# spcl/EBCC

Measured on AMD Instinct MI355X. Metric: fp32 GB/s encode+decode, 721x1440 ERA5 frames MAX_ERROR=0.5, higher is better.
Workload: dtype f32; 1 GPU; 256-frame batch 721x1440 fp32 per GPU, base_cr=30 MAX_ERROR=0.5 (BASELINE configs[1]); frames_per_gpu=256, parallelism=frames sharded over 1 GPU(s), no collective, hw_queues=4, encode_slices=3

## Files before the change

### ebcc_amd/csrc/j2k.hip

```cpp
#include <algorithm>
#include <cstring>
#include <vector>

#include "../../include/ebcc_hip.h"
#include "engine.hpp"
#include "j2k.hpp"

namespace ebcc {

bool j2k_create(ebcc_hip_ctx *ctx)
{
    J2kBuffers *jb = new J2kBuffers();
    ctx->j2k = jb;
    const int period = ctx->tile_period;
    std::vector<std::vector<J2kBlock>> tile_blocks((size_t) period);
    int stride = 0;
    for (int k = 0; k < period; k++) {
        jb->geoms.push_back(make_j2k_geom(ctx->height, ctx->width, tile_blocks[(size_t) k], k * ctx->height));
        stride = std::max(stride, jb->geoms.back().nblocks);
    }
    for (J2kGeom &t : jb->geoms) { t.period = period; t.stride = stride; }
    jb->geom = jb->geoms[0];
    const J2kGeom &g = jb->geom;
    const size_t n_pix = ctx->n_pix, F = ctx->max_frames;
    const size_t total = F * (size_t) stride, groups = (total + 63) / 64;
    jb->max_frames = (int) F;
    jb->fs = ctx->rb.fs;
    jb->stream_cap = ((n_pix * 3 + 4096 + 63) / 64) * 64;
    bool ok = true;
    ok &= (jb->d_geom = (J2kGeom *) ctx_alloc<uint8_t>(ctx, sizeof(J2kGeom) * (size_t) period)) != nullptr;
    ok &= (jb->d_blocks = (J2kBlock *) ctx_alloc<uint8_t>(ctx, sizeof(J2kBlock) * (size_t) period * (size_t) stride)) != nullptr;
    ok &= (jb->d_blkmap = ctx_alloc<uint16_t>(ctx, (size_t) period * n_pix)) != nullptr;
    ok &= (jb->B = ctx_alloc<float>(ctx, F * n_pix)) != nullptr;
    ok &= (jb->B2 = ctx_alloc<float>(ctx, F * n_pix)) != nullptr;
    ok &= (jb->Q6 = ctx_alloc<int32_t>(ctx, F * n_pix)) != nullptr;
    ok &= (jb->DEC = ctx_alloc<float>(ctx, F * n_pix)) != nullptr;
    ok &= (jb->V = ctx_alloc<int32_t>(ctx, F * n_pix)) != nullptr;
    ok &= (jb->BP = ctx_alloc<unsigned long long>(ctx, groups * kJ2kMaxPlanes * 64 * 64)) != nullptr;
    ok &= (jb->SGN = ctx_alloc<unsigned long long>(ctx, groups * 64 * 64)) != nullptr;
    ok &= (jb->SUF = ctx_alloc<unsigned long long>(ctx, groups * (kJ2kMaxPlanes + 2) * 64 * 64)) != nullptr;
    ok &= (jb->SPS = ctx_alloc<unsigned long long>(ctx, groups * 64 * 64)) != nullptr;
    ok &= (jb->VISP = ctx_alloc<unsigned long long>(ctx, groups * kJ2kMaxPlanes * 64 * 64)) != nullptr;
    ok &= (jb->ckpt = ctx_alloc<uint8_t>(ctx, groups * 64 * j2k_ckpt_block_bytes())) != nullptr;
    jb->SYM = nullptr;
    {
        const char *e = getenv("EBCC_T1_TWO_PHASE");
        jb->sym_rows = kJ2kSymRows;
        if (const char *r = getenv("EBCC_HIP_SYM_ROWS")) jb->sym_rows = std::max(1, std::min(kJ2kSymRows, atoi(r)));
        if (!e || atoi(e)) ok &= (jb->SYM = ctx_alloc<uint8_t>(ctx, groups * (size_t) ((jb->sym_rows + 1) & ~1) * 1024 + 256)) != nullptr;
    }
    ok &= (jb->seglen = ctx_alloc<uint16_t>(ctx, groups * (size_t) kJ2kSegCount * 64)) != nullptr;
    ok &= (jb->lanerows = ctx_alloc<uint32_t>(ctx, groups * 64)) != nullptr;
    ok &= (jb->qplane = (int *) ctx_alloc<int32_t>(ctx, groups * 64)) != nullptr;
    ok &= (jb->lastnp = (int *) ctx_alloc<int32_t>(ctx, groups * 64)) != nullptr;
    ok &= (jb->T1S = ctx_alloc<unsigned long long>(ctx, groups * kT1StateWords * 64)) != nullptr;
    ok &= (jb->blkmax = (int *) ctx_alloc<int32_t>(ctx, groups * 64)) != nullptr;
    ok &= (jb->numbps = (int *) ctx_alloc<int32_t>(ctx, groups * 64)) != nullptr;
    ok &= (jb->totalpasses = (int *) ctx_alloc<int32_t>(ctx, groups * 64)) != nullptr;
    ok &= (jb->cblk_len = (int *) ctx_alloc<int32_t>(ctx, groups * 64)) != nullptr;
    ok &= (jb->npass = (int *) ctx_alloc<int32_t>(ctx, groups * 64)) != nullptr;
    ok &= (jb->cand_cr = ctx_alloc<float>(ctx, F * 2)) != nullptr;
    ok &= (jb->cand_out = (int *) ctx_alloc<int32_t>(ctx, F * 6)) != nullptr;
    ok &= (jb->cand_npass = (int *) ctx_alloc<int32_t>(ctx, 2 * F * (size_t) stride)) != nullptr;
    ok &= (jb->cand_sel = (int *) ctx_alloc<int32_t>(ctx, F)) != nullptr;
    ok &= (jb->have_rate = (int *) ctx_alloc<int32_t>(ctx, F)) != nullptr;
    ok &= (jb->rate_path = (int *) ctx_alloc<int32_t>(ctx, F * 1536 * 3)) != nullptr;
    ok &= (jb->rate_path_n = (int *) ctx_alloc<int32_t>(ctx, 2 * F)) != nullptr;
    {
        int nodes = 0;
        for (const J2kGeom &t : jb->geoms) nodes = std::max(nodes, t.tree_nodes);
        J2kBuffers::RateCache &rc = jb->rate_cache;
        rc.nodes_cap = (nodes + 3) & ~3;
        rc.cap = stride * kJ2kMaxPasses;
        rc.ok = jb->rate_path_n ? jb->rate_path_n + F : nullptr;
        ok &= (rc.mnmx = ctx_alloc<double>(ctx, F * 2)) != nullptr;
        ok &= (rc.mval = (short *) ctx_alloc<uint16_t>(ctx, F * (size_t) rc.nodes_cap)) != nullptr;
        ok &= (rc.off = (int *) ctx_alloc<int32_t>(ctx, F * (size_t) (stride + 1))) != nullptr;
        ok &= (rc.crate = ctx_alloc<uint16_t>(ctx, F * (size_t) rc.cap)) != nullptr;
        ok &= (rc.cdisto = ctx_alloc<double>(ctx, F * (size_t) rc.cap)) != nullptr;
    }
    ok &= (jb->rates = (int *) ctx_alloc<int32_t>(ctx, groups * 64 * kJ2kMaxPasses)) != nullptr;
    ok &= (jb->disto = ctx_alloc<double>(ctx, groups * 64 * kJ2kMaxPasses)) != nullptr;
    ok &= (jb->cblk_bytes = ctx_alloc<uint8_t>(ctx, groups * 64 * kJ2kCblkBytes)) != nullptr;
    ok &= (jb->stream = ctx_alloc<uint8_t>(ctx, F * jb->stream_cap)) != nullptr;
    ok &= (jb->dec_table = (int *) ctx_alloc<int32_t>(ctx, groups * 64 * 4)) != nullptr;
    ok &= (jb->dec_order = (int *) ctx_alloc<int32_t>(ctx, groups * 64 + 128)) != nullptr;
    ok &= (jb->mq_order = (int *) ctx_alloc<int32_t>(ctx, groups * 64 + 256)) != nullptr;
    ok &= (jb->jf = (J2kFrame *) ctx_alloc<uint8_t>(ctx, sizeof(J2kFrame) * F)) != nullptr;
    ok &= (jb->partial = ctx_alloc<double>(ctx, F * kPartials)) != nullptr;
    ok &= (jb->partial_u = ctx_alloc<unsigned long long>(ctx, F * kPartials)) != nullptr;
    if (!ok) return false;
    poison_alloc(jb->cblk_bytes, groups * 64 * kJ2kCblkBytes);
    poison_alloc(jb->stream, F * jb->stream_cap);
    if (stride >= 65535) { set_error("too many code-blocks"); return false; }
    std::vector<uint16_t> map((size_t) period * n_pix, 0);
    std::vector<J2kBlock> blocks((size_t) period * (size_t) stride, J2kBlock{});
    for (int k = 0; k < period; k++) {
        const std::vector<J2kBlock> &tb = tile_blocks[(size_t) k];
        std::copy(tb.begin(), tb.end(), blocks.begin() + (size_t) k * (size_t) stride);
        for (size_t b = 0; b < tb.size(); b++)
            for (int y = 0; y < tb[b].h; y++)
                for (int x = 0; x < tb[b].w; x++) map[(size_t) k * n_pix + (size_t) (tb[b].y + y) * g.W + tb[b].x + x] = (uint16_t) b;
    }
    hipStream_t s = ctx->stream;
    EBCC_HIP_CHECK(hipMemcpyAsync(jb->d_geom, jb->geoms.data(), sizeof(J2kGeom) * (size_t) period, hipMemcpyHostToDevice, s));
    EBCC_HIP_CHECK(hipMemcpyAsync(jb->d_blocks, blocks.data(), sizeof(J2kBlock) * blocks.size(), hipMemcpyHostToDevice, s));
    EBCC_HIP_CHECK(hipMemcpyAsync(jb->d_blkmap, map.data(), map.size() * sizeof(uint16_t), hipMemcpyHostToDevice, s));
    EBCC_HIP_CHECK(hipHostMalloc(&ctx->h_jf, sizeof(J2kFrame) * F));
    EBCC_HIP_CHECK(hipHostMalloc((void **) &ctx->h_table, sizeof(int) * 4 * total));
    EBCC_HIP_CHECK(hipMemsetAsync(jb->jf, 0, sizeof(J2kFrame) * F, s));
    EBCC_HIP_CHECK(hipMemsetAsync(jb->rate_path_n, 0, sizeof(int) * 2 * F, s));
    wait_stream(s);
    return true;
}

void j2k_destroy(ebcc_hip_ctx *ctx)
{
    delete static_cast<J2kBuffers *>(ctx->j2k);
    ctx->j2k = nullptr;
    if (ctx->stream2) { hipStreamSynchronize(ctx->stream2); hipStreamDestroy(ctx->stream2); ctx->stream2 = nullptr; }
}

namespace {

struct BitReader {
    const uint8_t *p, *end;
// ... 478 lines not shown
```

### ebcc_amd/csrc/j2k.hpp

```cpp
#pragma once

#include <vector>

#include "../../include/ebcc_hip.h"
#include "common.hpp"
#include "residual.hpp"

namespace ebcc {

constexpr int kJ2kRes = 6;
constexpr int kJ2kBands = 3 * kJ2kRes - 2;
constexpr int kJ2kMaxPlanes = 26;
constexpr int kJ2kMaxPasses = 3 * kJ2kMaxPlanes;
constexpr int kJ2kCblkBytes = 16 * 1024;
constexpr int kT1StateWords = 66 + 4 * 64;

struct J2kBand {
    int res, orient, level;
    int x0, y0, x1, y1;
    int offx, offy;
    int ncw, nch;
    int first_block;
    int expn, mant, numbps;
    float step_enc, step_dec;
// ... 52 lines not shown
    float target;
    int maxlen;
    int body_bytes;
    int stream_bytes;
    unsigned long long nbad;
    double err_sum;
    int overflow;
    int keep;
    float hdr_share;
    unsigned int bad_limit;
    unsigned int bad_seen;
};

struct J2kBuffers {
    J2kGeom geom;
    std::vector<J2kGeom> geoms;
    J2kGeom *d_geom;
    J2kBlock *d_blocks;
    std::uint16_t *d_blkmap;
    int max_frames;
    float *B;
    float *B2;
    int32_t *Q6;
    float *DEC;
    unsigned long long *BP;
    unsigned long long *SGN;
    unsigned long long *SUF;
    unsigned long long *SPS;
    unsigned long long *VISP;
    void *ckpt;
    uint8_t *SYM;
    int sym_rows;
    std::uint16_t *seglen;
    std::uint32_t *lanerows;
    int *qplane;
    int *lastnp;
    unsigned long long *T1S;
    int *blkmax;
    int *numbps;
    int *totalpasses;
    int *cblk_len;
    int *rates;
    double *disto;
    int *npass;
    float *cand_cr;
    int *cand_out;
    int *cand_npass;
    int *cand_sel;
    int *have_rate;
    int *rate_path;
    int *rate_path_n;
    struct RateCache {
        int *ok;
        double *mnmx;
        short *mval;
        int *off;
        unsigned short *crate;
        double *cdisto;
        int nodes_cap, cap;
    } rate_cache;
    uint8_t *cblk_bytes;
    uint8_t *stream;
    size_t stream_cap;
    int32_t *V;
    int *dec_table;
    int *dec_order;
// ... 74 lines not shown
```

### ebcc_amd/csrc/j2k_analysis.hip

```cpp
#include <array>
#include <mutex>
#include <cmath>
#include <cstdlib>
#include <vector>

#include "j2k.hpp"
#include "t1_core.hpp"
#include "t1_device.hpp"

namespace ebcc {

static int ceildivpow2(int a, int b) { return (int) (((long long) a + (1ll << b) - 1) >> b); }
static int floorlog2i(int a) { int l = 0; while (a > 1) { a >>= 1; l++; } return l; }

static const double kNormsReal[4][10] = {
    {1.000, 1.965, 4.177, 8.403, 16.90, 33.84, 67.69, 135.3, 270.6, 540.9},
    {2.022, 3.989, 8.355, 17.04, 34.27, 68.63, 137.3, 274.6, 549.0},
    {2.022, 3.989, 8.355, 17.04, 34.27, 68.63, 137.3, 274.6, 549.0},
    {2.080, 3.865, 8.307, 17.18, 34.71, 69.59, 139.3, 278.6, 557.2}};

int t1_lanes_per_wave(int kernel, int total_blocks)
{
    int t[4] = {64, 64, 4, 2};
    if (const char *e = getenv("EBCC_T1_LPW")) {
// ... 1087 lines not shown

struct DevMasks {
    const unsigned char *bp, *suf, *sg;
    unsigned char *visp;
    uint32_t lane8;
    __device__ unsigned long long ld(const unsigned char *b, int row) const { return *(const unsigned long long *) (b + ((uint32_t) row * 512u + lane8)); }
    __device__ unsigned long long BP(int p, int y) const { return ld(bp, p * 64 + y); }
    __device__ unsigned long long SUF(int p, int y) const { return ld(suf, p * 64 + y); }
    __device__ unsigned long long SGN(int y) const { return ld(sg, y); }
    __device__ unsigned long long VISP(int p, int y) const { return ld(visp, p * 64 + y); }
};
struct Tier1Lane {
    int gid, frame, P, w, h, orient;
    bool live;
};
__device__ inline Tier1Lane tier1_lane(int gid, int total, const int *blkmax, const J2kGeom *geom, const J2kBlock *blocks, const FrameState *fs)
{
    Tier1Lane l{gid, 0, 0, 0, 0, 0, false};
    if (gid >= total) return l;
    const int nb = geom->stride;
    l.frame = gid / nb;
    if (fs[l.frame].const_field) return l;
    const J2kBlock blk = j2k_frame_blocks(geom, blocks, l.frame)[gid - l.frame * nb];
    const int m = blkmax[gid];
    l.P = m ? (31 - __clz(m)) + 1 - 6 : 0;
    l.w = blk.w; l.h = blk.h;
    l.orient = j2k_frame_geom(geom, l.frame).bands[blk.band].orient;
    l.live = l.P > 0;
    return l;
}

struct ScanOutDev {
    unsigned char *vp, *sp;
    std::uint16_t *lens;
    uint32_t lane8;
    __device__ void visp_row(unsigned char *b, int row, unsigned long long v) const { *(unsigned long long *) (b + ((uint32_t) row * 512u + lane8)) = v; }
    __device__ void visp(int p, int y, unsigned long long m) const { visp_row(vp, p * 64 + y, m); }
    __device__ void sps_or(int y, unsigned long long n) const { *(unsigned long long *) (sp + ((uint32_t) y * 512u + lane8)) |= n; }
    __device__ void len(int seg, uint32_t n) const { lens[(uint32_t) seg * 64u] = (std::uint16_t) n; }
};
__global__ __launch_bounds__(64) void k_t1_scan(const unsigned long long *BP, const unsigned long long *SUF, const unsigned long long *SGN,
                                                 unsigned long long *SPS, unsigned long long *VISP, const int *blkmax, int *numbps,
                                                 int *totalpasses, int *cblk_len, std::uint16_t *seglen, const J2kGeom *geom,
                                                 const J2kBlock *blocks, const FrameState *fs, int total)
{
    const size_t grp = blockIdx.x;
    const int gid = (int) (grp * 64) + (int) threadIdx.x;
    const Tier1Lane l = tier1_lane(gid, total, blkmax, geom, blocks, fs);
    if (gid < total) { numbps[gid] = l.P; totalpasses[gid] = l.live ? 3 * l.P - 2 : 0; cblk_len[gid] = 0; }
    if (!l.live) return;
    const uint32_t lane8 = threadIdx.x * 8u;
    DevMasks M{(const unsigned char *) (BP + grp * kJ2kMaxPlanes * 64 * 64), (const unsigned char *) (SUF + grp * (kJ2kMaxPlanes + 2) * 64 * 64),
               (const unsigned char *) (SGN + grp * 64 * 64), (unsigned char *) (VISP + grp * kJ2kMaxPlanes * 64 * 64), lane8};
    ScanOutDev out{M.visp, (unsigned char *) (SPS + grp * 64 * 64), seglen + grp * kJ2kSegCount * 64 + threadIdx.x, lane8};
    t1::scan_block(M, out, l.P, l.w, l.h, l.orient);
}

__global__ __launch_bounds__(64) void k_t1_rowoffs(std::uint16_t *seglen, uint32_t *lanerows, const int *blkmax, J2kFrame *jf,
                                                    const J2kGeom *geom, const J2kBlock *blocks, const FrameState *fs, int total,
                                                    uint32_t sym_rows)
{
    const size_t grp = blockIdx.x;
    const int gid = (int) (grp * 64) + (int) threadIdx.x;
    const Tier1Lane l = tier1_lane(gid, total, blkmax, geom, blocks, fs);
    std::uint16_t *L = seglen + grp * kJ2kSegCount * 64 + threadIdx.x;
    uint32_t off = 0;
    if (l.live) {
        const int nstr = (l.h + 3) >> 2;
        for (int seg0 = t1::seg_index(l.P - 1, 2, 0) & ~15; seg0 < kJ2kSegCount; seg0 += 16) {
            if (!t1::seg_valid(l.P, nstr, t1::seg_plane(seg0), t1::seg_type(seg0), 0)) continue;
            uint32_t n[16];
#pragma unroll
            for (int k = 0; k < 16; k++) n[k] = k < nstr ? L[(uint32_t) (seg0 + k) * 64u] : 0u;
#pragma unroll
            for (int k = 0; k < 16; k++)
                if (k < nstr) { L[(uint32_t) (seg0 + k) * 64u] = (std::uint16_t) off; off += t1::seg_rows(n[k]); }
        }
    }
    if (gid < total) lanerows[gid] = off;
    if (off > sym_rows) atomicOr(&jf[l.frame].overflow, 2);
}

__device__ inline size_t sym_row_offset(uint32_t row) { return (size_t) (row >> 1) * 2048 + (size_t) (row & 1u) * 16; }
__host__ __device__ inline size_t sym_group_bytes(uint32_t sym_rows) { return (size_t) ((sym_rows + 1u) & ~1u) * 1024; }
struct SegEmDev {
    unsigned char *ring;
    uint8_t *sym;
    const std::uint16_t *rowoff;
    uint32_t cap;
    uint32_t cnt = 0, fl = 0;
    uint32_t row0 = 0;
    __device__ void begin(int seg) { cnt = 0; fl = 0; row0 = rowoff[(uint32_t) seg * 64u]; }
    __device__ void emit_if(bool on, uint32_t ctx, uint32_t d)
    {
        ring[cnt & 63u] = (unsigned char) (ctx | (d << 5));
        cnt += on ? 1u : 0u;
    }
    __device__ void piece(uint32_t keep)
    {
        const uint32_t *q = (const uint32_t *) (ring + ((fl & 3u) << 4));
        uint32_t w[4] = {q[0], q[1], q[2], q[3]};
        if (keep < 16u) {
#pragma unroll
            for (int d = 0; d < 4; d++) {
                const int nv = min(max((int) keep - 4 * d, 0), 4);
                const uint32_t m = nv ? 0xFFFFFFFFu >> (32 - 8 * nv) : 0u;
                w[d] = (w[d] & m) | ((t1::kRowPad * 0x01010101u) & ~m);
            }
        }
        if (fl == 0) w[0] |= t1::kRowStart;
        if (row0 + fl < cap) *(uint4 *) (sym + sym_row_offset(row0 + fl)) = make_uint4(w[0], w[1], w[2], w[3]);
        fl++;
    }
    __device__ void column_end() { if ((cnt >> 4) != fl) piece(16u); }
    __device__ void end()
    {
        if ((cnt >> 4) != fl) piece(16u);
        if ((cnt & 15u) || cnt == 0) piece(cnt & 15u);
    }
};

__global__ __launch_bounds__(64) void k_t1_emit(const unsigned long long *BP, const unsigned long long *SUF, const unsigned long long *SGN,
                                                 unsigned long long *VISP, const int *blkmax, uint8_t *SYM, const std::uint16_t *seglen,
                                                 const uint32_t *lanerows, const J2kGeom *geom, const J2kBlock *blocks,
                                                 const FrameState *fs, int total, uint32_t sym_rows)
{
    __shared__ uint32_t ring[17 * 64];
    const size_t grp = blockIdx.x;
    const int p = (int) blockIdx.y;
    const int gid = (int) (grp * 64) + (int) threadIdx.x;
    const Tier1Lane l = tier1_lane(gid, total, blkmax, geom, blocks, fs);
    if (!l.live || p >= l.P || lanerows[gid] > sym_rows) return;
    const uint32_t lane8 = threadIdx.x * 8u;
    DevMasks M{(const unsigned char *) (BP + grp * kJ2kMaxPlanes * 64 * 64), (const unsigned char *) (SUF + grp * (kJ2kMaxPlanes + 2) * 64 * 64),
               (const unsigned char *) (SGN + grp * 64 * 64), (unsigned char *) (VISP + grp * kJ2kMaxPlanes * 64 * 64), lane8};
    SegEmDev em{(unsigned char *) ring + threadIdx.x * 68u, SYM + grp * sym_group_bytes(sym_rows) + threadIdx.x * 32u,
                seglen + grp * kJ2kSegCount * 64 + threadIdx.x, sym_rows};
    const int nstr = (l.h + 3) >> 2;
    for (int s = 0; s < nstr; s++) t1::emit_stripe_segments(M, em, l.P, p, s, l.w, l.h, l.orient);
}

constexpr int kRowChunk = 2;
struct RowSrcDev {
    uint32_t buf;
    uint32_t n, wn;
    __device__ uint32_t rows() const { return n; }
    __device__ uint32_t wave_rows() const { return wn; }
    __device__ void sync(uint32_t row) const { if (row % kRowChunk == 0) __syncthreads(); }
    __device__ void finish() const { __syncthreads(); __syncthreads(); }
    __device__ void load(uint32_t row, uint32_t w[4]) const
    {
        typedef uint32_t u32x4 __attribute__((ext_vector_type(4)));
        const u32x4 v = *(const __attribute__((address_space(3))) u32x4 *) (uintptr_t) (buf + (row % (2 * kRowChunk)) * 1024u);
        w[0] = v.x; w[1] = v.y; w[2] = v.z; w[3] = v.w;
    }
};
struct HandDev {
    uint32_t buf;
    __device__ void put(uint32_t row, int j, uint32_t word) const
    {
        *(__attribute__((address_space(3))) uint32_t *) (uintptr_t) (buf + ((row % (2 * kRowChunk)) * 16u + (uint32_t) j) * 256u) = word;
    }
    __device__ uint32_t get(uint32_t row, int j) const
    {
        return *(const __attribute__((address_space(3))) uint32_t *) (uintptr_t) (buf + ((row % (2 * kRowChunk)) * 16u + (uint32_t) j) * 256u);
    }
};
struct MqSinkLds {
    unsigned char *ring;
    uint8_t *out; int *overflow;
    int fl = 0;
    __device__ void put(int i, uint32_t b) { ring[(uint32_t) i & 63u] = (unsigned char) b; }
    __device__ void sector()
    {
        const uint32_t *q = (const uint32_t *) (ring + ((uint32_t) fl & 63u));
        if (fl + 32 <= kJ2kCblkBytes) {
            uint4 *o = (uint4 *) (out + fl);
            o[0] = make_uint4(q[0], q[1], q[2], q[3]);
            o[1] = make_uint4(q[4], q[5], q[6], q[7]);
        } else *overflow = 1;
        fl += 32;
    }
    __device__ void row_end(int n) { while (fl + 32 <= n) sector(); }
    __device__ void finish(int n) { row_end(n); if (fl < n) sector(); }
};

constexpr int kMqClasses = 128;
__device__ inline int mq_class(uint32_t rows, uint32_t sym_rows) { return rows == 0 || rows > sym_rows ? 0 : min(kMqClasses - 1, 1 + (int) (rows >> 5)); }
__global__ __launch_bounds__(256) void k_mq_hist(const uint32_t *lanerows, int *counters, int total, uint32_t sym_rows)
{
    __shared__ int h[kMqClasses];
    if (threadIdx.x < kMqClasses) h[threadIdx.x] = 0;
    __syncthreads();
    const int gid = blockIdx.x * blockDim.x + threadIdx.x;
    if (gid < total) atomicAdd(&h[mq_class(lanerows[gid], sym_rows)], 1);
    __syncthreads();
    if (threadIdx.x < kMqClasses && h[threadIdx.x]) atomicAdd(&counters[threadIdx.x], h[threadIdx.x]);
}
__global__ void k_mq_offsets(int *counters)
{
    const int c = threadIdx.x;
    int before = 0;
    for (int k = kMqClasses - 1; k > c; k--) before += counters[k];
    counters[kMqClasses + c] = before;
}
__global__ __launch_bounds__(256) void k_mq_place(const uint32_t *lanerows, int *counters, int *order, int total, int padded, uint32_t sym_rows)
{
    __shared__ int h[kMqClasses], base[kMqClasses];
    if (threadIdx.x < kMqClasses) h[threadIdx.x] = 0;
    __syncthreads();
    const int gid = blockIdx.x * blockDim.x + threadIdx.x;
    int cls = 0, rank = 0;
    if (gid < total) { cls = mq_class(lanerows[gid], sym_rows); rank = atomicAdd(&h[cls], 1); }
    __syncthreads();
    if (threadIdx.x < kMqClasses && h[threadIdx.x]) base[threadIdx.x] = atomicAdd(&counters[kMqClasses + threadIdx.x], h[threadIdx.x]);
    __syncthreads();
    if (gid < total) order[base[cls] + rank] = gid;
    else if (gid < padded) order[gid] = -1;
}

__global__ __launch_bounds__(128) void k_t1_mqrows(const uint8_t *SYM, const uint32_t *lanerows, const int *blkmax, int *cblk_len,
                                                    int *rates, uint8_t *cblk_bytes, void *ckpt, const J2kGeom *geom,
                                                    const J2kBlock *blocks, const FrameState *fs, J2kFrame *jf, int total, uint32_t sym_rows,
                                                    const int *order)
{
    __shared__ uint2 tab_store[128];
    __shared__ uint32_t ctxw[CtxSlotsLds::kBytes / 4];
    __shared__ uint32_t bring[17 * 64];
    __shared__ uint4 rowbuf[2 * kRowChunk * 64];
    __shared__ uint32_t handbuf[2 * kRowChunk * 16 * 64];
    __shared__ uint32_t a_end[64];
// ... 174 lines not shown
            h[2 * 128 + i] = (short) std::max(0, x);
            x = (int) (std::floor((u * u) * std::pow(2, 6) + 0.5) / std::pow(2, 6) * 8192.0);
            h[3 * 128 + i] = (short) std::max(0, x);
        }
        EBCC_HIP_CHECK(device_malloc((void **) &g_luts, sizeof h));
        EBCC_HIP_CHECK(hipMemcpyAsync(g_luts, h, sizeof h, hipMemcpyHostToDevice, s));
        wait_stream(s);
    }
    return g_luts;
}

__global__ void k_jf_reset(J2kFrame *jf, int n)
{
    const int f = blockIdx.x * blockDim.x + threadIdx.x;
    if (f < n) jf[f].overflow = 0;
}

void launch_j2k_tier1(const J2kBuffers &jb, int n_frames, hipStream_t s, bool single_kernel)
{
    const J2kGeom &g = jb.geom;
    const FrameState *fs = jb.fs;
    const int total = n_frames * g.stride;
    const size_t groups = ((size_t) total + 63) / 64;
    EBCC_HIP_CHECK(hipMemsetAsync(jb.SPS, 0, groups * 64 * 64 * sizeof(unsigned long long), s));
    timing_begin("t1_encode", s);
    if (!jb.SYM || single_kernel) {
        EBCC_HIP_CHECK(hipMemsetAsync(jb.T1S, 0, groups * kT1StateWords * 64 * sizeof(unsigned long long), s));
        int lpw = getenv("EBCC_T1_LPW") ? t1_lanes_per_wave(T1_ENCODE) : 32;
        unsigned t1_grid = (unsigned) ceil_div(total, lpw);
        hipLaunchKernelGGL(k_t1_encode, dim3(t1_grid), dim3(64), 0, s, jb.T1S, jb.BP, jb.SGN, jb.SPS, jb.blkmax, jb.numbps,
                           jb.totalpasses, jb.cblk_len, jb.rates, jb.cblk_bytes, jb.ckpt, jb.VISP, jb.d_geom,
                           jb.d_blocks, fs, jb.jf, total, lpw);
    } else {
        EBCC_HIP_CHECK(hipMemsetAsync(jb.seglen, 0, groups * (size_t) kJ2kSegCount * 64 * sizeof(std::uint16_t), s));
        timing_begin("t1_symbols", s);
        hipLaunchKernelGGL(k_t1_scan, dim3((unsigned) groups), dim3(64), 0, s, jb.BP, jb.SUF, jb.SGN, jb.SPS, jb.VISP, jb.blkmax, jb.numbps,
                           jb.totalpasses, jb.cblk_len, jb.seglen, jb.d_geom, jb.d_blocks, fs, total);
        hipLaunchKernelGGL(k_t1_rowoffs, dim3((unsigned) groups), dim3(64), 0, s, jb.seglen, jb.lanerows, jb.blkmax, jb.jf, jb.d_geom, jb.d_blocks,
                           fs, total, (uint32_t) jb.sym_rows);
        hipLaunchKernelGGL(k_t1_emit, dim3((unsigned) groups, kJ2kMaxPlanes), dim3(64), 0, s, jb.BP, jb.SUF, jb.SGN, jb.VISP, jb.blkmax, jb.SYM,
                           jb.seglen, jb.lanerows, jb.d_geom, jb.d_blocks, fs, total, (uint32_t) jb.sym_rows);
        timing_end("t1_symbols", s);
        if (getenv("EBCC_HIP_T1_STATS")) {
            std::vector<uint32_t> tot((size_t) total);
            EBCC_HIP_CHECK(hipMemcpyAsync(tot.data(), jb.lanerows, sizeof(uint32_t) * (size_t) total, hipMemcpyDeviceToHost, s));
            wait_stream(s);
            uint32_t mx = 0; double sum = 0, wsum = 0;
            for (size_t g0 = 0; g0 < (size_t) total; g0 += 64) {
                uint32_t wm = 0;
                for (size_t i = g0; i < std::min((size_t) total, g0 + 64); i++) { wm = std::max(wm, tot[i]); sum += tot[i]; }
                wsum += wm; mx = std::max(mx, wm);
            }
            fprintf(stderr, "ebcc-mi355x tier-1: %zu groups, rows of 16 decisions: per code-block mean %.0f, per wave mean %.0f max %u (cap %d)\n", groups,
                    sum / (double) total, wsum / (double) groups, mx, jb.sym_rows);
        }
        timing_begin("t1_mq", s);
        const int *order = nullptr;
        if (!getenv("EBCC_HIP_MQ_NATURAL_ORDER")) {
            int *counters = jb.mq_order + groups * 64;
            EBCC_HIP_CHECK(hipMemsetAsync(counters, 0, 2 * kMqClasses * sizeof(int), s));
            hipLaunchKernelGGL(k_mq_hist, dim3(ceil_div(total, 256)), dim3(256), 0, s, jb.lanerows, counters, total, (uint32_t) jb.sym_rows);
            hipLaunchKernelGGL(k_mq_offsets, dim3(1), dim3(kMqClasses), 0, s, counters);
            hipLaunchKernelGGL(k_mq_place, dim3(ceil_div((int) (groups * 64), 256)), dim3(256), 0, s, jb.lanerows, counters, jb.mq_order, total, (int) (groups * 64),
                               (uint32_t) jb.sym_rows);
            order = jb.mq_order;
        }
        hipLaunchKernelGGL(k_t1_mqrows, dim3((unsigned) groups), dim3(128), 0, s, jb.SYM, jb.lanerows, jb.blkmax, jb.cblk_len, jb.rates,
                           jb.cblk_bytes, jb.ckpt, jb.d_geom, jb.d_blocks, fs, jb.jf, total, (uint32_t) jb.sym_rows, order);
        timing_end("t1_mq", s);
    }
    timing_end("t1_encode", s);
    hipLaunchKernelGGL(k_distortion, dim3(g.stride, n_frames), dim3(256), 0, s, jb.Q6, jb.SPS, jb.numbps, jb.totalpasses,
                       jb.disto, nmsedec_luts(s), jb.d_geom, jb.d_blocks, fs);
    EBCC_HIP_LAUNCH_CHECK();
}

bool j2k_tier1_retry(const J2kBuffers &jb, int n_frames, const J2kFrame *host_jf, hipStream_t s)
{
    bool need = false;
    for (int f = 0; f < n_frames; f++) need |= (host_jf[f].overflow & 2) != 0;
    if (!need) return false;
    hipLaunchKernelGGL(k_jf_reset, dim3(ceil_div(n_frames, 64)), dim3(64), 0, s, jb.jf, n_frames);
    launch_j2k_tier1(jb, n_frames, s, true);
    return true;
}

constexpr int kFwdT = 64;
__global__ __launch_bounds__(kFwdT) void k_j2k_cols_fwd_top(const float *__restrict__ data, float *__restrict__ B, const J2kGeom *geom,
                                                             const FrameState *fs)
{
    const int frame = blockIdx.y;
    if (fs[frame].const_field) return;
    const J2kGeom &g = j2k_frame_geom(geom, frame);
    constexpr int r = kJ2kRes - 1;
    const int W = g.W, nv = g.rh[r], sn = g.rh[r - 1], dn = nv - sn;
    const int col = blockIdx.x * kFwdT + threadIdx.x;
    if (col >= g.rw[r]) return;
    const size_t n_pix = (size_t) W * g.H;
    const float *x = data + (size_t) frame * n_pix + col;
// ... 194 lines not shown
```

### ebcc_amd/csrc/t1_core.hpp

```cpp
#pragma once

#include <cstdint>
#include <type_traits>

#if defined(__HIPCC__)
#define T1_HD __host__ __device__ inline
#else
#define T1_HD inline
#endif
#ifndef T1_STAT
#define T1_STAT(i)
#endif

namespace ebcc {
namespace t1 {

typedef unsigned long long u64;

enum { CTX_ZC0 = 0, CTX_SC0 = 9, CTX_MAG0 = 14, CTX_AGG = 17, CTX_UNI = 18, NCTX = 19 };
constexpr int kMaxPasses = 3 * 30;

T1_HD uint32_t mq_entry(int i)
{
    constexpr uint32_t T[47] = {
// ... 1134 lines not shown
    rates[p] = n;
    int last = n;
    for (int q = npasses; q > 0;) {
        --q;
        if (rates[q] > last) rates[q] = last; else last = rates[q];
    }
    for (int q = 0; q < npasses; q++)
        if (rates[q] > 0 && bytes(rates[q] - 1) == 0xFF) rates[q]--;
    EncodeResult r;
    r.totalpasses = npasses;
    r.length = n;
    return r;
}

constexpr int kSegPlanes = 26;
constexpr int kSegCount = kSegPlanes * 3 * 16;
T1_HD int seg_index(int p, int t, int s) { return ((kSegPlanes - 1 - p) * 3 + t) * 16 + s; }
T1_HD int seg_plane(int seg) { return kSegPlanes - 1 - seg / 48; }
T1_HD int seg_type(int seg) { return (seg >> 4) % 3; }
T1_HD bool seg_valid(int P, int nstr, int p, int t, int s) { return p < P && (p < P - 1 || t == 2) && s < nstr; }

template <class Masks>
struct MaskRows {
    Masks &M;
    int h;
    T1_HD u64 bp(int p, int y) const { return (y >= 0 && y < h) ? M.BP(p, y) : 0ull; }
    T1_HD u64 suf(int p, int y) const { return (y >= 0 && y < h) ? M.SUF(p, y) : 0ull; }
    T1_HD u64 sgn(int y) const { return (y >= 0 && y < h) ? M.SGN(y) : 0ull; }
    T1_HD u64 visp(int p, int y) const { return (y >= 0 && y < h) ? M.VISP(p, y) : 0ull; }
};
struct NullCoder {};

template <class Masks, class Out>
T1_HD void scan_block(Masks &M, Out &out, int P, int w, int h, int orient)
{
    NullCoder nc;
    Passes<true, Masks, NullCoder> ps(M, nc, w, h, orient);
    const MaskRows<Masks> R{M, h};
    const int nstr = (h + 3) >> 2;
    for (int p = P - 1; p >= 0; p--) {
        const bool top = p == P - 1;
        Stripe sp;
        sp.wmask = w >= 64 ? ~0ull : ((1ull << w) - 1);
        if (!top) {
            u64 carry = 0;
            for (int s = 0; s < nstr; s++) {
                const int y0 = 4 * s;
                sp.nrows = h - y0 < 4 ? h - y0 : 4;
#pragma unroll
                for (int r = 0; r < 6; r++) sp.s[r] = R.suf(p + 1, y0 - 1 + r);
                const u64 b[4] = {R.bp(p, y0), R.bp(p, y0 + 1), R.bp(p, y0 + 2), R.bp(p, y0 + 3)};
                const uint32_t nref = (uint32_t) (ps.popc64(sp.s[1]) + ps.popc64(sp.s[2]) + ps.popc64(sp.s[3]) + ps.popc64(sp.s[4]));
                sp.s[0] |= carry;
                u64 m[4], n[4];
                ps.sigprop_members(sp, b, m, n);
#pragma unroll
                for (int r = 0; r < 4; r++)
                    if (r < sp.nrows) { out.visp(p, y0 + r, m[r]); if (n[r]) out.sps_or(y0 + r, n[r]); }
                out.len(seg_index(p, 0, s), ps.sigprop_count(m, n));
                out.len(seg_index(p, 1, s), nref);
                carry = n[3];
            }
        }
        for (int s = 0; s < nstr; s++) {
            const int y0 = 4 * s;
            sp.nrows = h - y0 < 4 ? h - y0 : 4;
            sp.s[0] = R.suf(p, y0 - 1);
#pragma unroll
            for (int r = 1; r < 6; r++) {
                const int y = y0 - 1 + r;
                sp.s[r] = R.suf(p + 1, y) | (top ? 0ull : (R.visp(p, y) & R.bp(p, y)));
            }
#pragma unroll
            for (int r = 0; r < 4; r++) sp.vis[r] = top ? 0ull : R.visp(p, y0 + r);
            const u64 b[4] = {R.bp(p, y0), R.bp(p, y0 + 1), R.bp(p, y0 + 2), R.bp(p, y0 + 3)};
            u64 m[4], n[4], agg;
            ps.cleanup_members(sp, b, y0 + 3 < h, m, n, agg);
            out.len(seg_index(p, 2, s), ps.cleanup_count(m, n, b, agg));
        }
    }
}

template <class Masks, class Em>
T1_HD void emit_stripe_segments(Masks &M, Em &em, int P, int p, int s, int w, int h, int orient)
{
    Passes<true, Masks, Em> ps(M, em, w, h, orient);
    const MaskRows<Masks> R{M, h};
    const bool top = p == P - 1;
    const int y0 = 4 * s;
    u64 s1[6], A[6], sg[6], vp[6];
#pragma unroll
    for (int r = 0; r < 6; r++) {
        const int y = y0 - 1 + r;
        s1[r] = R.suf(p + 1, y);
        sg[r] = R.sgn(y);
        vp[r] = top ? 0ull : R.visp(p, y);
        A[r] = s1[r] | (vp[r] & R.bp(p, y));
    }
    const u64 b[4] = {R.bp(p, y0), R.bp(p, y0 + 1), R.bp(p, y0 + 2), R.bp(p, y0 + 3)};
    Stripe sp;
    sp.wmask = w >= 64 ? ~0ull : ((1ull << w) - 1);
    sp.nrows = h - y0 < 4 ? h - y0 : 4;
#pragma unroll
    for (int r = 0; r < 4; r++) { sp.sgn[r] = sg[r + 1]; sp.sps[r] = 0; }
    u64 m[4], n[4];
    if (!top) {
        sp.s[0] = A[0];
#pragma unroll
        for (int r = 1; r < 6; r++) sp.s[r] = s1[r];
#pragma unroll
        for (int r = 0; r < 6; r++) sp.neg[r] = sp.s[r] & sg[r];
#pragma unroll
        for (int r = 0; r < 4; r++) sp.vis[r] = 0;
// ... 30 lines not shown
T1_HD uint32_t mq_code_state(uint32_t code) { return code >> 3; }
T1_HD void mq_entry2(int st7, uint32_t &qe, uint32_t &next)
{
    const int i = st7 & 63, mps = st7 >> 6;
    if (i >= 47) { qe = 0; next = kNullCode | (kNullCode << 16); return; }
    const uint32_t e = mq_entry(i);
    const uint32_t nm = ((e >> 16) & 0x3Fu) | ((uint32_t) mps << 6), nl = ((e >> 22) & 0x3Fu) | (((uint32_t) mps ^ (e >> 28)) << 6);
    qe = e & 0xFFFFu;
    next = mq_code(nm) | (mq_code(nl) << 16);
}
struct ConstTable2 {
    T1_HD void operator()(uint32_t code, uint32_t &qe, uint32_t &next) const { mq_entry2((int) mq_code_state(code), qe, next); }
};
T1_HD uint32_t mq_slot_word(uint32_t code)
{
    uint32_t qe, nxt;
    mq_entry2((int) mq_code_state(code), qe, nxt);
    return qe | (code << 16);
}
T1_HD void mq_entry_next(uint32_t code, uint32_t &nxt, uint32_t &nqes)
{
    uint32_t qe, qm, ql, t;
    mq_entry2((int) mq_code_state(code), qe, nxt);
    mq_entry2((int) mq_code_state(nxt & 0xFFFFu), qm, t);
    mq_entry2((int) mq_code_state(nxt >> 16), ql, t);
    nqes = qm | (ql << 16);
}
struct ConstTableNext {
    T1_HD void operator()(uint32_t code, uint32_t &nxt, uint32_t &nqes) const { mq_entry_next(code, nxt, nqes); }
};

constexpr uint32_t kRowPad = 0x80u | kCtxNull, kRowStart = 0x40u;
T1_HD uint32_t seg_rows(uint32_t decisions) { return decisions ? (decisions + 15u) >> 4 : 1u; }

constexpr uint32_t kHandNoAdd = 1u << 20, kHandStart = 1u << 21;

template <class RowSrc, class Slots, class Hand, class CkArray, class Table = ConstTableNext>
T1_HD uint32_t mq_rows_interval(RowSrc src, Slots cx, int P, int nstr, Hand hand, CkArray &ck, Table tab = Table())
{
    uint32_t a = 0x8000, shifts = 0;
    for (uint32_t i = 0; i <= kCtxNull; i++)
        cx.st(cx.handle(i), mq_slot_word(i >= (uint32_t) NCTX ? kNullCode : mq_code(i == CTX_UNI ? 46u : (i == CTX_AGG ? 3u : (i == CTX_ZC0 ? 4u : 0u)))));
    const uint32_t nrows = P > 0 ? src.rows() : 0u, wrows = src.wave_rows();
    int pass = 0, stripe = 0;
    for (uint32_t row = 0; row < wrows; row++) {
        src.sync(row);
        if (row < nrows) {
            uint32_t w[4];
            src.load(row, w);
            const bool start = (w[0] & kRowStart) != 0;
            if (start) {
                uint32_t x[5];
                cx.words(x);
                ck.store_interval(pass, stripe, a, shifts, x);
                if (++stripe == nstr) { stripe = 0; pass++; }
            }
            uint32_t h = cx.handle(w[0] & 31u);
            uint32_t s0 = cx.ld(h);
            uint32_t nxt, nqes;
            tab(s0 >> 16, nxt, nqes);
#pragma unroll
            for (int j = 0; j < 16; j++) {
                const uint32_t wj = w[j >> 2] >> (8 * (j & 3));
                uint32_t hn = 0, sn = 0;
                if (j < 15) {
                    hn = cx.handle((w[(j + 1) >> 2] >> (8 * ((j + 1) & 3))) & 31u);
// ... 157 lines not shown
```

Baseline: 8.941 GB/s.

## Parallelize T1 scan across bit-planes and fuse MQ histogram into rowoffs

The per-block T1 scan kernel now launches one workgroup per (group, bit-plane) instead of looping over all planes serially in one lane. Each plane computes local segment row offsets in shared memory and writes a per-plane row total. The row-offset kernel then does only a short prefix over plane totals and also builds the MQ class histogram, which removes the separate histogram kernel and the seglen memset. Because planes now run concurrently, the significance-propagation OR needs an atomicOr, and many workgroups exit early for planes at or above P.

Measured after the change: 8.973 GB/s (median of 3 runs). No clear change (+0.4%).

```diff
diff --git a/ebcc_amd/csrc/j2k.hip b/ebcc_amd/csrc/j2k.hip
--- a/ebcc_amd/csrc/j2k.hip
+++ b/ebcc_amd/csrc/j2k.hip
@@ -49,7 +49,8 @@
         if (const char *r = getenv("EBCC_HIP_SYM_ROWS")) jb->sym_rows = std::max(1, std::min(kJ2kSymRows, atoi(r)));
         if (!e || atoi(e)) ok &= (jb->SYM = ctx_alloc<uint8_t>(ctx, groups * (size_t) ((jb->sym_rows + 1) & ~1) * 1024 + 256)) != nullptr;
     }
-    ok &= (jb->seglen = ctx_alloc<uint16_t>(ctx, groups * (size_t) kJ2kSegCount * 64)) != nullptr;
+    ok &= (jb->seglen = ctx_alloc<uint16_t>(ctx, groups * (size_t) (kJ2kSegCount + kJ2kMaxPlanes) * 64)) != nullptr;
+    jb->planerows = jb->seglen ? jb->seglen + groups * (size_t) kJ2kSegCount * 64 : nullptr;
     ok &= (jb->lanerows = ctx_alloc<uint32_t>(ctx, groups * 64)) != nullptr;
     ok &= (jb->qplane = (int *) ctx_alloc<int32_t>(ctx, groups * 64)) != nullptr;
     ok &= (jb->lastnp = (int *) ctx_alloc<int32_t>(ctx, groups * 64)) != nullptr;
@@ -92,6 +93,8 @@
     if (!ok) return false;
     poison_alloc(jb->cblk_bytes, groups * 64 * kJ2kCblkBytes);
     poison_alloc(jb->stream, F * jb->stream_cap);
+    poison_alloc(jb->seglen, groups * (size_t) (kJ2kSegCount + kJ2kMaxPlanes) * 64 * sizeof(uint16_t));
+    poison_alloc(jb->lanerows, groups * 64 * sizeof(uint32_t));
     if (stride >= 65535) { set_error("too many code-blocks"); return false; }
     std::vector<uint16_t> map((size_t) period * n_pix, 0);
     std::vector<J2kBlock> blocks((size_t) period * (size_t) stride, J2kBlock{});
diff --git a/ebcc_amd/csrc/j2k.hpp b/ebcc_amd/csrc/j2k.hpp
--- a/ebcc_amd/csrc/j2k.hpp
+++ b/ebcc_amd/csrc/j2k.hpp
@@ -108,6 +108,7 @@
     uint8_t *SYM;
     int sym_rows;
     std::uint16_t *seglen;
+    std::uint16_t *planerows;
     std::uint32_t *lanerows;
     int *qplane;
     int *lastnp;
diff --git a/ebcc_amd/csrc/j2k_analysis.hip b/ebcc_amd/csrc/j2k_analysis.hip
--- a/ebcc_amd/csrc/j2k_analysis.hip
+++ b/ebcc_amd/csrc/j2k_analysis.hip
@@ -1143,53 +1143,67 @@
 
 struct ScanOutDev {
     unsigned char *vp, *sp;
-    std::uint16_t *lens;
+    std::uint16_t *cnt;
+    int seg0;
     uint32_t lane8;
     __device__ void visp_row(unsigned char *b, int row, unsigned long long v) const { *(unsigned long long *) (b + ((uint32_t) row * 512u + lane8)) = v; }
     __device__ void visp(int p, int y, unsigned long long m) const { visp_row(vp, p * 64 + y, m); }
-    __device__ void sps_or(int y, unsigned long long n) const { *(unsigned long long *) (sp + ((uint32_t) y * 512u + lane8)) |= n; }
-    __device__ void len(int seg, uint32_t n) const { lens[(uint32_t) seg * 64u] = (std::uint16_t) n; }
+    __device__ void sps_or(int y, unsigned long long n) const { atomicOr((unsigned long long *) (sp + ((uint32_t) y * 512u + lane8)), n); }
+    __device__ void len(int seg, uint32_t n) const { cnt[(uint32_t) (seg - seg0) * 64u] = (std::uint16_t) n; }
 };
 __global__ __launch_bounds__(64) void k_t1_scan(const unsigned long long *BP, const unsigned long long *SUF, const unsigned long long *SGN,
                                                  unsigned long long *SPS, unsigned long long *VISP, const int *blkmax, int *numbps,
-                                                 int *totalpasses, int *cblk_len, std::uint16_t *seglen, const J2kGeom *geom,
-                                                 const J2kBlock *blocks, const FrameState *fs, int total)
-{
+                                                 int *totalpasses, int *cblk_len, std::uint16_t *seglen, std::uint16_t *planerows,
+                                                 const J2kGeom *geom, const J2kBlock *blocks, const FrameState *fs, int total)
+{
+    __shared__ std::uint16_t cnt[48 * 64];
     const size_t grp = blockIdx.x;
+    const int p = (int) blockIdx.y;
     const int gid = (int) (grp * 64) + (int) threadIdx.x;
     const Tier1Lane l = tier1_lane(gid, total, blkmax, geom, blocks, fs);
-    if (gid < total) { numbps[gid] = l.P; totalpasses[gid] = l.live ? 3 * l.P - 2 : 0; cblk_len[gid] = 0; }
-    if (!l.live) return;
+    if (p == 0 && gid < total) { numbps[gid] = l.P; totalpasses[gid] = l.live ? 3 * l.P - 2 : 0; cblk_len[gid] = 0; }
+    if (!l.live || p >= l.P) return;
     const uint32_t lane8 = threadIdx.x * 8u;
     DevMasks M{(const unsigned char *) (BP + grp * kJ2kMaxPlanes * 64 * 64), (const unsigned char *) (SUF + grp * (kJ2kMaxPlanes + 2) * 64 * 64),
                (const unsigned char *) (SGN + grp * 64 * 64), (unsigned char *) (VISP + grp * kJ2kMaxPlanes * 64 * 64), lane8};
-    ScanOutDev out{M.visp, (unsigned char *) (SPS + grp * 64 * 64), seglen + grp * kJ2kSegCount * 64 + threadIdx.x, lane8};
-    t1::scan_block(M, out, l.P, l.w, l.h, l.orient);
-}
-
-__global__ __launch_bounds__(64) void k_t1_rowoffs(std::uint16_t *seglen, uint32_t *lanerows, const int *blkmax, J2kFrame *jf,
-                                                    const J2kGeom *geom, const J2kBlock *blocks, const FrameState *fs, int total,
-                                                    uint32_t sym_rows)
-{
-    const size_t grp = blockIdx.x;
-    const int gid = (int) (grp * 64) + (int) threadIdx.x;
+    const int seg0 = t1::seg_index(p, 0, 0);
+    ScanOutDev out{M.visp, (unsigned char *) (SPS + grp * 64 * 64), cnt + threadIdx.x, seg0, lane8};
+    t1::scan_plane(M, out, l.P, p, l.w, l.h, l.orient);
+    std::uint16_t *L = seglen + (grp * kJ2kSegCount + (size_t) seg0) * 64 + threadIdx.x;
+    const std::uint16_t *c = cnt + threadIdx.x;
+    const uint32_t rows = t1::plane_row_offsets(l.P, (l.h + 3) >> 2, p, [c](int t, int s) { return (uint32_t) c[(uint32_t) (t * 16 + s) * 64u]; },
+                                                [L](int t, int s, uint32_t row) { L[(uint32_t) (t * 16 + s) * 64u] = (std::uint16_t) row; });
+    planerows[(grp * kJ2kMaxPlanes + (size_t) p) * 64 + threadIdx.x] = (std::uint16_t) rows;
+}
+
+constexpr int kMqClasses = 128;
+__device__ inline int mq_class(uint32_t rows, uint32_t sym_rows) { return rows == 0 || rows > sym_rows ? 0 : min(kMqClasses - 1, 1 + (int) (rows >> 5)); }
+__global__ __launch_bounds__(256) void k_t1_rowoffs(std::uint16_t *planerows, uint32_t *lanerows, const int *blkmax, J2kFrame *jf,
+                                                     const J2kGeom *geom, const J2kBlock *blocks, const FrameState *fs, int total,
+                                                     uint32_t sym_rows, int *counters)
+{
+    __shared__ int h[kMqClasses];
+    if (threadIdx.x < kMqClasses) h[threadIdx.x] = 0;
+    __syncthreads();
+    const int gid = blockIdx.x * blockDim.x + threadIdx.x;
     const Tier1Lane l = tier1_lane(gid, total, blkmax, geom, blocks, fs);
-    std::uint16_t *L = seglen + grp * kJ2kSegCount * 64 + threadIdx.x;
     uint32_t off = 0;
     if (l.live) {
-        const int nstr = (l.h + 3) >> 2;
-        for (int seg0 = t1::seg_index(l.P - 1, 2, 0) & ~15; seg0 < kJ2kSegCount; seg0 += 16) {
-            if (!t1::seg_valid(l.P, nstr, t1::seg_plane(seg0), t1::seg_type(seg0), 0)) continue;
-            uint32_t n[16];
+        std::uint16_t *R = planerows + ((size_t) (gid >> 6) * kJ2kMaxPlanes * 64 + (size_t) (gid & 63));
+        uint32_t n[kJ2kMaxPlanes];
 #pragma unroll
-            for (int k = 0; k < 16; k++) n[k] = k < nstr ? L[(uint32_t) (seg0 + k) * 64u] : 0u;
+        for (int k = 0; k < kJ2kMaxPlanes; k++) n[k] = k < l.P ? R[(uint32_t) k * 64u] : 0u;
 #pragma unroll
-            for (int k = 0; k < 16; k++)
-                if (k < nstr) { L[(uint32_t) (seg0 + k) * 64u] = (std::uint16_t) off; off += t1::seg_rows(n[k]); }
-        }
-    }
-    if (gid < total) lanerows[gid] = off;
+        for (int k = kJ2kMaxPlanes - 1; k >= 0; k--)
+            if (k < l.P) { R[(uint32_t) k * 64u] = (std::uint16_t) off; off += n[k]; }
+    }
+    if (gid < total) {
+        lanerows[gid] = off;
+        if (counters) atomicAdd(&h[mq_class(off, sym_rows)], 1);
+    }
     if (off > sym_rows) atomicOr(&jf[l.frame].overflow, 2);
+    __syncthreads();
+    if (counters && threadIdx.x < kMqClasses && h[threadIdx.x]) atomicAdd(&counters[threadIdx.x], h[threadIdx.x]);
 }
 
 __device__ inline size_t sym_row_offset(uint32_t row) { return (size_t) (row >> 1) * 2048 + (size_t) (row & 1u) * 16; }
@@ -1198,10 +1212,11 @@
     unsigned char *ring;
     uint8_t *sym;
     const std::uint16_t *rowoff;
+    uint32_t base;
     uint32_t cap;
     uint32_t cnt = 0, fl = 0;
     uint32_t row0 = 0;
-    __device__ void begin(int seg) { cnt = 0; fl = 0; row0 = rowoff[(uint32_t) seg * 64u]; }
+    __device__ void begin(int seg) { cnt = 0; fl = 0; row0 = base + rowoff[(uint32_t) seg * 64u]; }
     __device__ void emit_if(bool on, uint32_t ctx, uint32_t d)
     {
         ring[cnt & 63u] = (unsigned char) (ctx | (d << 5));
@@ -1233,7 +1248,7 @@
 
 __global__ __launch_bounds__(64) void k_t1_emit(const unsigned long long *BP, const unsigned long long *SUF, const unsigned long long *SGN,
                                                  unsigned long long *VISP, const int *blkmax, uint8_t *SYM, const std::uint16_t *seglen,
-                                                 const uint32_t *lanerows, const J2kGeom *geom, const J2kBlock *blocks,
+                                                 const std::uint16_t *planerows, const uint32_t *lanerows, const J2kGeom *geom, const J2kBlock *blocks,
                                                  const FrameState *fs, int total, uint32_t sym_rows)
 {
     __shared__ uint32_t ring[17 * 64];
@@ -1246,7 +1261,7 @@
     DevMasks M{(const unsigned char *) (BP + grp * kJ2kMaxPlanes * 64 * 64), (const unsigned char *) (SUF + grp * (kJ2kMaxPlanes + 2) * 64 * 64),
                (const unsigned char *) (SGN + grp * 64 * 64), (unsigned char *) (VISP + grp * kJ2kMaxPlanes * 64 * 64), lane8};
     SegEmDev em{(unsigned char *) ring + threadIdx.x * 68u, SYM + grp * sym_group_bytes(sym_rows) + threadIdx.x * 32u,
-                seglen + grp * kJ2kSegCount * 64 + threadIdx.x, sym_rows};
+                seglen + grp * kJ2kSegCount * 64 + threadIdx.x, planerows[(grp * kJ2kMaxPlanes + (size_t) p) * 64 + threadIdx.x], sym_rows};
     const int nstr = (l.h + 3) >> 2;
     for (int s = 0; s < nstr; s++) t1::emit_stripe_segments(M, em, l.P, p, s, l.w, l.h, l.orient);
 }
@@ -1296,18 +1311,6 @@
     __device__ void finish(int n) { row_end(n); if (fl < n) sector(); }
 };
 
-constexpr int kMqClasses = 128;
-__device__ inline int mq_class(uint32_t rows, uint32_t sym_rows) { return rows == 0 || rows > sym_rows ? 0 : min(kMqClasses - 1, 1 + (int) (rows >> 5)); }
-__global__ __launch_bounds__(256) void k_mq_hist(const uint32_t *lanerows, int *counters, int total, uint32_t sym_rows)
-{
-    __shared__ int h[kMqClasses];
-    if (threadIdx.x < kMqClasses) h[threadIdx.x] = 0;
-    __syncthreads();
-    const int gid = blockIdx.x * blockDim.x + threadIdx.x;
-    if (gid < total) atomicAdd(&h[mq_class(lanerows[gid], sym_rows)], 1);
-    __syncthreads();
-    if (threadIdx.x < kMqClasses && h[threadIdx.x]) atomicAdd(&counters[threadIdx.x], h[threadIdx.x]);
-}
 __global__ void k_mq_offsets(int *counters)
 {
     const int c = threadIdx.x;
@@ -1548,14 +1551,25 @@
                            jb.totalpasses, jb.cblk_len, jb.rates, jb.cblk_bytes, jb.ckpt, jb.VISP, jb.d_geom,
                            jb.d_blocks, fs, jb.jf, total, lpw);
     } else {
-        EBCC_HIP_CHECK(hipMemsetAsync(jb.seglen, 0, groups * (size_t) kJ2kSegCount * 64 * sizeof(std::uint16_t), s));
         timing_begin("t1_symbols", s);
-        hipLaunchKernelGGL(k_t1_scan, dim3((unsigned) groups), dim3(64), 0, s, jb.BP, jb.SUF, jb.SGN, jb.SPS, jb.VISP, jb.blkmax, jb.numbps,
-                           jb.totalpasses, jb.cblk_len, jb.seglen, jb.d_geom, jb.d_blocks, fs, total);
-        hipLaunchKernelGGL(k_t1_rowoffs, dim3((unsigned) groups), dim3(64), 0, s, jb.seglen, jb.lanerows, jb.blkmax, jb.jf, jb.d_geom, jb.d_blocks,
-                           fs, total, (uint32_t) jb.sym_rows);
+        const int *order = nullptr;
+        int *counters = nullptr;
+        if (!getenv("EBCC_HIP_MQ_NATURAL_ORDER")) {
+            counters = jb.mq_order + groups * 64;
+            EBCC_HIP_CHECK(hipMemsetAsync(counters, 0, 2 * kMqClasses * sizeof(int), s));
+            order = jb.mq_order;
+        }
+        hipLaunchKernelGGL(k_t1_scan, dim3((unsigned) groups, kJ2kMaxPlanes), dim3(64), 0, s, jb.BP, jb.SUF, jb.SGN, jb.SPS, jb.VISP, jb.blkmax, jb.numbps,
+                           jb.totalpasses, jb.cblk_len, jb.seglen, jb.planerows, jb.d_geom, jb.d_blocks, fs, total);
+        hipLaunchKernelGGL(k_t1_rowoffs, dim3(ceil_div(total, 256)), dim3(256), 0, s, jb.planerows, jb.lanerows, jb.blkmax, jb.jf, jb.d_geom, jb.d_blocks,
+                           fs, total, (uint32_t) jb.sym_rows, counters);
+        if (order) {
+            hipLaunchKernelGGL(k_mq_offsets, dim3(1), dim3(kMqClasses), 0, s, counters);
+            hipLaunchKernelGGL(k_mq_place, dim3(ceil_div((int) (groups * 64), 256)), dim3(256), 0, s, jb.lanerows, counters, jb.mq_order, total, (int) (groups * 64),
+                               (uint32_t) jb.sym_rows);
+        }
         hipLaunchKernelGGL(k_t1_emit, dim3((unsigned) groups, kJ2kMaxPlanes), dim3(64), 0, s, jb.BP, jb.SUF, jb.SGN, jb.VISP, jb.blkmax, jb.SYM,
-                           jb.seglen, jb.lanerows, jb.d_geom, jb.d_blocks, fs, total, (uint32_t) jb.sym_rows);
+                           jb.seglen, jb.planerows, jb.lanerows, jb.d_geom, jb.d_blocks, fs, total, (uint32_t) jb.sym_rows);
         timing_end("t1_symbols", s);
         if (getenv("EBCC_HIP_T1_STATS")) {
             std::vector<uint32_t> tot((size_t) total);
@@ -1571,16 +1585,6 @@
                     sum / (double) total, wsum / (double) groups, mx, jb.sym_rows);
         }
         timing_begin("t1_mq", s);
-        const int *order = nullptr;
-        if (!getenv("EBCC_HIP_MQ_NATURAL_ORDER")) {
-            int *counters = jb.mq_order + groups * 64;
-            EBCC_HIP_CHECK(hipMemsetAsync(counters, 0, 2 * kMqClasses * sizeof(int), s));
-            hipLaunchKernelGGL(k_mq_hist, dim3(ceil_div(total, 256)), dim3(256), 0, s, jb.lanerows, counters, total, (uint32_t) jb.sym_rows);
-            hipLaunchKernelGGL(k_mq_offsets, dim3(1), dim3(kMqClasses), 0, s, counters);
-            hipLaunchKernelGGL(k_mq_place, dim3(ceil_div((int) (groups * 64), 256)), dim3(256), 0, s, jb.lanerows, counters, jb.mq_order, total, (int) (groups * 64),
-                               (uint32_t) jb.sym_rows);
-            order = jb.mq_order;
-        }
         hipLaunchKernelGGL(k_t1_mqrows, dim3((unsigned) groups), dim3(128), 0, s, jb.SYM, jb.lanerows, jb.blkmax, jb.cblk_len, jb.rates,
                            jb.cblk_bytes, jb.ckpt, jb.d_geom, jb.d_blocks, fs, jb.jf, total, (uint32_t) jb.sym_rows, order);
         timing_end("t1_mq", s);
diff --git a/ebcc_amd/csrc/t1_core.hpp b/ebcc_amd/csrc/t1_core.hpp
--- a/ebcc_amd/csrc/t1_core.hpp
+++ b/ebcc_amd/csrc/t1_core.hpp
@@ -1190,53 +1190,56 @@
 struct NullCoder {};
 
 template <class Masks, class Out>
-T1_HD void scan_block(Masks &M, Out &out, int P, int w, int h, int orient)
+T1_HD void scan_plane(Masks &M, Out &out, int P, int p, int w, int h, int orient)
 {
     NullCoder nc;
     Passes<true, Masks, NullCoder> ps(M, nc, w, h, orient);
     const MaskRows<Masks> R{M, h};
     const int nstr = (h + 3) >> 2;
-    for (int p = P - 1; p >= 0; p--) {
-        const bool top = p == P - 1;
-        Stripe sp;
-        sp.wmask = w >= 64 ? ~0ull : ((1ull << w) - 1);
-        if (!top) {
-            u64 carry = 0;
-            for (int s = 0; s < nstr; s++) {
-                const int y0 = 4 * s;
-                sp.nrows = h - y0 < 4 ? h - y0 : 4;
-#pragma unroll
-                for (int r = 0; r < 6; r++) sp.s[r] = R.suf(p + 1, y0 - 1 + r);
-                const u64 b[4] = {R.bp(p, y0), R.bp(p, y0 + 1), R.bp(p, y0 + 2), R.bp(p, y0 + 3)};
-                const uint32_t nref = (uint32_t) (ps.popc64(sp.s[1]) + ps.popc64(sp.s[2]) + ps.popc64(sp.s[3]) + ps.popc64(sp.s[4]));
-                sp.s[0] |= carry;
-                u64 m[4], n[4];
-                ps.sigprop_members(sp, b, m, n);
-#pragma unroll
-                for (int r = 0; r < 4; r++)
-                    if (r < sp.nrows) { out.visp(p, y0 + r, m[r]); if (n[r]) out.sps_or(y0 + r, n[r]); }
-                out.len(seg_index(p, 0, s), ps.sigprop_count(m, n));
-                out.len(seg_index(p, 1, s), nref);
-                carry = n[3];
-            }
-        }
+    const bool top = p == P - 1;
+    Stripe sp;
+    sp.wmask = w >= 64 ? ~0ull : ((1ull << w) - 1);
+    if (!top) {
+        u64 carry = 0;
         for (int s = 0; s < nstr; s++) {
             const int y0 = 4 * s;
             sp.nrows = h - y0 < 4 ? h - y0 : 4;
-            sp.s[0] = R.suf(p, y0 - 1);
-#pragma unroll
-            for (int r = 1; r < 6; r++) {
-                const int y = y0 - 1 + r;
-                sp.s[r] = R.suf(p + 1, y) | (top ? 0ull : (R.visp(p, y) & R.bp(p, y)));
-            }
-#pragma unroll
-            for (int r = 0; r < 4; r++) sp.vis[r] = top ? 0ull : R.visp(p, y0 + r);
+#pragma unroll
+            for (int r = 0; r < 6; r++) sp.s[r] = R.suf(p + 1, y0 - 1 + r);
             const u64 b[4] = {R.bp(p, y0), R.bp(p, y0 + 1), R.bp(p, y0 + 2), R.bp(p, y0 + 3)};
-            u64 m[4], n[4], agg;
-            ps.cleanup_members(sp, b, y0 + 3 < h, m, n, agg);
-            out.len(seg_index(p, 2, s), ps.cleanup_count(m, n, b, agg));
-        }
-    }
+            const uint32_t nref = (uint32_t) (ps.popc64(sp.s[1]) + ps.popc64(sp.s[2]) + ps.popc64(sp.s[3]) + ps.popc64(sp.s[4]));
+            sp.s[0] |= carry;
+            u64 m[4], n[4];
+            ps.sigprop_members(sp, b, m, n);
+#pragma unroll
+            for (int r = 0; r < 4; r++)
+                if (r < sp.nrows) { out.visp(p, y0 + r, m[r]); if (n[r]) out.sps_or(y0 + r, n[r]); }
+            out.len(seg_index(p, 0, s), ps.sigprop_count(m, n));
+            out.len(seg_index(p, 1, s), nref);
+            carry = n[3];
+        }
+    }
+    for (int s = 0; s < nstr; s++) {
+        const int y0 = 4 * s;
+        sp.nrows = h - y0 < 4 ? h - y0 : 4;
+        sp.s[0] = R.suf(p, y0 - 1);
+#pragma unroll
+        for (int r = 1; r < 6; r++) {
+            const int y = y0 - 1 + r;
+            sp.s[r] = R.suf(p + 1, y) | (top ? 0ull : (R.visp(p, y) & R.bp(p, y)));
+        }
+#pragma unroll
+        for (int r = 0; r < 4; r++) sp.vis[r] = top ? 0ull : R.visp(p, y0 + r);
+        const u64 b[4] = {R.bp(p, y0), R.bp(p, y0 + 1), R.bp(p, y0 + 2), R.bp(p, y0 + 3)};
+        u64 m[4], n[4], agg;
+        ps.cleanup_members(sp, b, y0 + 3 < h, m, n, agg);
+        out.len(seg_index(p, 2, s), ps.cleanup_count(m, n, b, agg));
+    }
+}
+template <class Masks, class Out>
+T1_HD void scan_block(Masks &M, Out &out, int P, int w, int h, int orient)
+{
+    for (int p = P - 1; p >= 0; p--) scan_plane(M, out, P, p, w, h, orient);
 }
 
 template <class Masks, class Em>
@@ -1333,6 +1336,17 @@
 
 constexpr uint32_t kRowPad = 0x80u | kCtxNull, kRowStart = 0x40u;
 T1_HD uint32_t seg_rows(uint32_t decisions) { return decisions ? (decisions + 15u) >> 4 : 1u; }
+template <class Cnt, class Put>
+T1_HD uint32_t plane_row_offsets(int P, int nstr, int p, Cnt cnt, Put put)
+{
+    uint32_t off = 0;
+    for (int t = p == P - 1 ? 2 : 0; t < 3; t++)
+        for (int s = 0; s < nstr; s++) {
+            put(t, s, off);
+            off += seg_rows(cnt(t, s));
+        }
+    return off;
+}
 
 constexpr uint32_t kHandNoAdd = 1u << 20, kHandStart = 1u << 21;
 
```
